# DixianZhu/deBWT

Hardware: AMD Instinct MI355X
Metric: Gbp/sec BWT build (30 Gbp synthetic DNA); bit-exact vs CPU ref; 1/2/4/8-GPU (higher is better)
Workload: dtype u64

## Files before the change

### debwt_amd/csrc/debwt_hip.hip

```cpp
#include "../../include/debwt_hip.h"

#include <hip/hip_runtime.h>

#include <algorithm>
#include <new>
#include <chrono>
#include <cmath>
#include <cstdio>
#include <cstring>
#include <atomic>
#include <string>
#include <thread>
#include <tuple>
#include <vector>

#include "radix_sort.h"
#include "special_host.h"
#include "fasta_host.h"
#include "gz_parallel.h"
#include "stage_kernels.h"
#include "special_kernels.h"
#include "verify_kernels.h"
#include "fm_kernels.h"
#include "fm_search_kernels.h"
// ... 1027 lines not shown
    }
    if ((rc = sync_check(c))) return rc;
    c->rB = c->h_scalars[4];
    c->rnlarge = c->h_scalars[5];
    c->rn1024 = c->h_scalars[11];
    c->rn512 = c->h_scalars[12];
    return DEBWT_OK;
}

static int append_range(debwt_ctx *c, debwt_ctx::KeyRange &r) {
    const u64 Q = c->rQ, nf = c->Rmo + Q;
    r.Q = Q; r.qbase = c->Q; r.B = c->rB; r.Bbase = c->B; r.l0 = c->nlarge; r.nl = c->rnlarge;
    ENSURE_KEEP(c, c->facts_acc, (c->nfacts_acc + nf) * 8 + 64, c->nfacts_acc * 8);
    ENSURE_KEEP(c, c->blk_j0, (c->Q + Q) * 8 + 64, c->Q * 8);
    ENSURE_KEEP(c, c->blk_freq, (c->Q + Q) * 4 + 64, c->Q * 4);
    ENSURE_KEEP(c, c->blk_start, (c->Q + Q) * 8 + 64, c->Q * 8);
    ENSURE_KEEP(c, c->large_q, (c->nlarge + c->rnlarge) * 4 + 64, c->nlarge * 4);
    if (nf) HIPCHK(c, hipMemcpyAsync(c->facts_acc.as<u64>() + c->nfacts_acc, c->facts.p, nf * 8, hipMemcpyDeviceToDevice, c->stream));
    if (Q)
        k_append_blocks<<<grid_for(Q, 256), 256, 0, c->stream>>>(c->mi_j0.as<u32>(), c->mi_freq.as<u32>(), c->bstart.as<u32>(), Q,
                                                                 r.Mbase, r.Bbase, c->blk_j0.as<u64>() + r.qbase,
                                                                 c->blk_freq.as<u32>() + r.qbase, c->blk_start.as<u64>() + r.qbase);
    if (c->rnlarge) {
        HIPCHK(c, hipMemcpyAsync(c->large_q.as<u32>() + c->nlarge, c->large_tmp.p, c->rnlarge * 4, hipMemcpyDeviceToDevice, c->stream));
        if (r.qbase)
            k_offset_u32<<<grid_for(c->rnlarge, 256), 256, 0, c->stream>>>(c->large_q.as<u32>() + c->nlarge, c->rnlarge, (u32)r.qbase);
    }
    c->nfacts_acc += nf; c->Q += Q; c->B += c->rB; c->nlarge += c->rnlarge; c->n1024 += c->rn1024; c->n512 += c->rn512;
    if (c->Q >= 0xFFFFFFF0ull) { c->err = "more than 2^32 multi-in blocks"; return DEBWT_ERANGE; }
    c->facts_ready = true;
    return sync_check(c);
}

static int classify_global(debwt_ctx *c, const u64 *d_facts, u64 nfacts, u64 qbase, u64 btotal) {
    const u64 nrec = c->nrec, Q = c->Q;
    int rc;
    const u64 nf = nfacts + nrec;
    c->nfacts = nf;
    c->qbase = qbase;
    c->Btotal = btotal;
    ENSURE(c, c->facts_all, nf * 8 + 64);
    ENSURE(c, c->facts_tmp, nf * 8 + 64);
    ENSURE(c, c->rs_skew, (nf / 2048 + 2) * 4);
    ENSURE(c, c->red, nf * 8 + 64);
    ENSURE(c, c->red_q, nf * 4 + 64);
    u64 *all = c->facts_all.as<u64>();
    if (nfacts) HIPCHK(c, hipMemcpyAsync(all, d_facts, nfacts * 8, hipMemcpyDeviceToDevice, c->stream));
    if (c->special_dev) HIPCHK(c, hipMemcpyAsync(all + nfacts, c->tail_d.p, nrec * 8, hipMemcpyDeviceToDevice, c->stream));
    else HIPCHK(c, hipMemcpyAsync(all + nfacts, c->special.tail_facts.data(), nrec * 8, hipMemcpyHostToDevice, c->stream));
    u64 *sorted_facts = nullptr;
    if ((rc = sort_keys(c, all, c->facts_tmp.as<u64>(), nf, 2 * c->cfg.k, &sorted_facts, false))) return rc;
    RedUniqueF fr{sorted_facts, nf, c->red.as<u64>()};
    if ((rc = cp_count(c, fr, nf, cp_area(c, 3), 3))) return rc;
    if ((rc = cp_emit(c, fr, nf, cp_area(c, 3)))) return rc;
    if ((rc = sync_check(c))) return rc;
    c->R = c->h_scalars[3];
    const u64 R = c->R;
    RedBlockF fq{c->red.as<u64>(), c->red_q.as<u32>()};
    if ((rc = cp_count(c, fq, R, cp_area(c, 6), 6))) return rc;
    if ((rc = cp_emit(c, fq, R, cp_area(c, 6)))) return rc;
    ENSURE(c, c->blue, c->B * 8 + 64);
    if ((rc = sync_check(c))) return rc;
    if (c->shard_world == 1 && c->h_scalars[6] != Q) {
        c->err = "multi-in count mismatch between fact list and red table";
        return DEBWT_EINTERNAL;
    }
    c->st.red_capacity = R; c->st.blue_capacity = c->B; c->st.blue_bound_num = Q; c->st.case3num = 2 * Q;
    c->st.blue_large_blocks = c->nlarge;
    c->Qtotal = c->h_scalars[6];
    c->stage = ST_CLASSIFIED;
    return DEBWT_OK;
}

extern "C" int debwt_classify(debwt_ctx *c) {
    if (!c) return DEBWT_EINVAL;
    if (c->stage < ST_SORTED) return DEBWT_ESTATE;
    if (c->shard_world > 1) { c->err = "sharded context: use debwt_shard_classify_local/_global"; return DEBWT_ESTATE; }
    HIPCHK(c, hipSetDevice(c->cfg.device));
    int rc;
    if (!c->local_done) {
        c->Q = c->B = c->nlarge = 0; c->nfacts_acc = 0; c->n1024 = 0; c->n512 = 0;
        if ((rc = classify_local(c))) return rc;
        if ((rc = append_range(c, c->ranges[0]))) return rc;
    }
    return classify_global(c, c->facts_acc.as<u64>(), c->nfacts_acc, 0, c->B);
}


static int sp_prepare(debwt_ctx *c) {
    HIPCHK(c, hipEventRecord(c->ev[4], c->stream));
    struct ReclaimScope { debwt_ctx *c; ~ReclaimScope() { c->reclaim_ok = false; } } rscope{c};
    c->reclaim_ok = true;
    const u64 ngroups = (c->n + 31) >> 5;
    ENSURE(c, c->momask, ngroups * 4 + 64);
    ENSURE(c, c->mimask, ngroups * 4 + 64);
    int hbits = 10;
    u64 slots_per_node = 4;
    if (const char *e = getenv("DEBWT_NODE_SLOTS")) slots_per_node = std::max<u64>(2, strtoull(e, nullptr, 10));
    while ((1ull << hbits) < slots_per_node * c->R) hbits++;
    if (hbits > 32 && (1ull << 32) >= 2 * c->R) hbits = 32;
    c->mzfilter = c->K >= 16 && !(c->cfg.reserved & 2048) && (hbits >= 20 || (c->cfg.reserved & 4096));
    c->mzw = c->K >= 24 ? MZ_W : MZ_W_SHORT;
    c->mztable = c->mzfilter && c->K >= 24 && (c->cfg.reserved & 16384);
    int pb;
    if (c->mzfilter) {
        pb = 10;
        while ((2ull << pb) < c->R) pb++;
        if (c->cfg.reserved & 15) pb += (c->cfg.reserved & 15) - 8;
        if (pb < 10) pb = 10;
        if (pb > 30) pb = 30;
    } else {
        pb = (c->cfg.reserved & 15) ? hbits + (c->cfg.reserved & 15) - 8
                                     : (hbits <= 24 ? std::max(hbits, std::min(hbits + 3, 24)) : hbits + 3);
        if (pb < 10) pb = 10;
        if (pb > 31) pb = 31;
    }
    if (pb > 31 || hbits > 32) { c->err = "more than 2^31 branching nodes: the node table has 2^32 slots"; return DEBWT_ERANGE; }
    c->hbits = hbits; c->pbits = pb;
    c->abs32 = c->B < 0xFFFFFFF0ull && !(c->cfg.reserved & 16);
    size_t rb_bytes = (c->mzfilter ? ((size_t)8 << pb) : ((size_t)1 << pb) / 8) + 64, ht_slots = (size_t)1 << hbits;
    ENSURE(c, c->rbits, rb_bytes);
    ENSURE(c, c->htab, ht_slots * sizeof(HSlot));
    HIPCHK(c, hipMemsetAsync(c->rbits.p, 0, rb_bytes, c->stream));
    HIPCHK(c, hipMemsetAsync(c->htab.p, 0, ht_slots * sizeof(HSlot), c->stream));
    if (c->R) {
        k_build_hash<<<grid_for(c->R, 256), 256, 0, c->stream>>>(c->red.as<u64>(), c->R, c->red_q.as<u32>(),
                                                                c->blk_start.as<u64>(), c->abs32 ? 1 : 0, (u32)c->qbase,
                                                                (u32)c->Q, hbits, c->htab.as<HSlot>(), c->mzfilter ? 0 : pb,
                                                                c->rbits.as<u32>(), c->mztable ? c->K : 0);
        if (c->mzfilter)
            k_build_mzfilter<<<grid_for(c->R, 256), 256, 0, c->stream>>>(c->red.as<u64>(), c->R, c->K, pb, c->rbits.as<u64>(), c->mzw);
    }
    return DEBWT_OK;
}

#define SP_SLICE_GROUPS (1ull << 26)
static SpBlockIds sp_block_ids(debwt_ctx *c) {
    if (!c->route_direct) return SpBlockIds{nullptr, nullptr, nullptr, 0};
    return SpBlockIds{c->qlist.as<u32>(), c->qwave.as<unsigned long long>(), c->qwave.as<u64>() + 1, c->gq0};
}
static int sp_block_ids_begin(debwt_ctx *c, u64 gq0, u64 groups) {
    c->route_direct = true; c->gq0 = gq0;
    ENSURE(c, c->qlist, (std::min<u64>(groups * 32, c->Btotal) + 64) * 4);
    ENSURE(c, c->qwave, ((groups + 63) / 64 + 2) * 8);
    HIPCHK(c, hipMemsetAsync(c->qwave.p, 0, 8, c->stream));
    return DEBWT_OK;
}

static int sp_flags(debwt_ctx *c, u64 g0, u64 g1) {
    int rc;
    if (g1 - g0 > (1ull << 27) - 2) { c->err = "text slice of the SP stage exceeds 2^32 positions"; return DEBWT_ERANGE; }
    c->g0 = g0; c->g1 = g1;
    const u64 ng = g1 - g0;
    if (ng && c->mzfilter && c->mztable)
        k_sp_flags<2><<<grid_for(ng, DEBWT_BLOCK), DEBWT_BLOCK, 0, c->stream>>>(
            c->text.as<u64>(), c->sepbits.as<u64>(), c->n, c->K, c->htab.as<HSlot>(), c->hbits, c->rbits.as<u32>(), c->pbits,
            c->branch.as<u64>(), c->nbranch, c->momask.as<u32>(), c->mimask.as<u32>(), g0, g1,
            sp_block_ids(c), c->branch_bitmap ? c->brbits.as<u64>() : nullptr);
    else if (ng && c->mzfilter)
        k_sp_flags<1><<<grid_for(ng, DEBWT_BLOCK), DEBWT_BLOCK, 0, c->stream>>>(
            c->text.as<u64>(), c->sepbits.as<u64>(), c->n, c->K, c->htab.as<HSlot>(), c->hbits, c->rbits.as<u32>(), c->pbits,
            c->branch.as<u64>(), c->nbranch, c->momask.as<u32>(), c->mimask.as<u32>(), g0, g1,
            sp_block_ids(c), c->branch_bitmap ? c->brbits.as<u64>() : nullptr, c->mzw);
    else if (ng)
        k_sp_flags<0><<<grid_for(ng, DEBWT_BLOCK), DEBWT_BLOCK, 0, c->stream>>>(
            c->text.as<u64>(), c->sepbits.as<u64>(), c->n, c->K, c->htab.as<HSlot>(), c->hbits, c->rbits.as<u32>(), c->pbits,
            c->branch.as<u64>(), c->nbranch, c->momask.as<u32>(), c->mimask.as<u32>(), g0, g1,
            sp_block_ids(c), c->branch_bitmap ? c->brbits.as<u64>() : nullptr);
    SpCountF fc{c->momask.as<u32>() + g0, c->mimask.as<u32>() + g0};
    if ((rc = cp_count2(c, fc, ng, cp_area(c, 0), 8, cp_area(c, 1), 10))) return rc;
    if ((rc = sync_check(c))) return rc;
    c->S_local = c->h_scalars[8];
    c->B_slice = c->h_scalars[10];
    return DEBWT_OK;
}

static int sp_emit(debwt_ctx *c, u64 sp_off, u64 *routed = nullptr, int qshift = 0) {
    const u64 ng = c->g1 - c->g0;
    c->sp_off = sp_off;
    ENSURE_KEEP(c, c->spsym, sp_off + c->S_local + 64, c->shard_world > 1 ? 0 : sp_off);
    if (!routed) ENSURE(c, c->mi_list, c->B_slice * 16 + 64);
    if (ng) {
        SpEmitArgs ea{c->text.as<u64>(), c->sepbits.as<u64>(), c->n, c->K, c->momask.as<u32>(), c->mimask.as<u32>(),
                      c->spsym.as<u8>(), routed ? nullptr : c->mi_list.as<ulonglong2>(), c->g0, sp_off,
                      routed, qshift, sp_block_ids(c)};
        u32 nchunks; u64 chunk;
        plan_chunks(ng, &nchunks, &chunk);
        k_sp_emit<<<nchunks, DEBWT_BLOCK, 0, c->stream>>>(ea, ng, chunk, cp_area(c, 0), cp_area(c, 1));
    }
    return DEBWT_OK;
}

static int sp_finish(debwt_ctx *c, u64 S) {
    c->S = S;
    u64 ntriples = (S >> 6) + 3;
    ENSURE(c, c->spn, ntriples * 24);
    k_pack_sp<<<grid_for(ntriples, 256), 256, 0, c->stream>>>(c->spsym.as<u8>(), S, ntriples, c->spn.as<u64>());
    c->st.sp_len = S;
    c->stage = ST_SP;
    return DEBWT_OK;
}

extern "C" int debwt_sp_generate(debwt_ctx *c) {
    if (!c) return DEBWT_EINVAL;
    if (c->stage < ST_CLASSIFIED) return DEBWT_ESTATE;
    HIPCHK(c, hipSetDevice(c->cfg.device));
    int rc;
    if ((rc = sp_prepare(c))) return rc;
    const u64 ngroups = (c->n + 31) >> 5;
    const u64 slice_groups = (c->cfg.reserved & 4194304) ? 4096ull : SP_SLICE_GROUPS;
    u64 S = 0, Bseen = 0;
    int qbits = 1;
    while ((1ull << qbits) < c->Q) qbits++;
    const int qshift = 64 - qbits;
    const bool route_sort = c->shard_world == 1 && c->Q > 0 && c->n < (1ull << (qshift - 3)) &&
                            c->B < 0xFFFFFFF0ull - (1ull << 20) &&
                            !(c->cfg.reserved & 32) &&
                            !((c->cfg.reserved & 262144) && c->ranges.size() > 1);
    const size_t P = c->ranges.size();
    bool route_ranges = !route_sort && c->shard_world == 1 && P > 1 && P <= RS_RADIX && c->Q > 0 && c->n < (1ull << (qshift - 3)) &&
                        !(c->cfg.reserved & 32);
    for (size_t i = 0; route_ranges && i < P; i++) route_ranges = c->ranges[i].B < 0xFFFFFFF0ull - (1ull << 20);
    std::vector<u64> rfill(P, 0), roffs(P + 1, 0);
    if (route_ranges) {
        std::vector<u32> qb(P + 1);
        for (size_t i = 0; i < P; i++) qb[i] = (u32)c->ranges[i].qbase;
        qb[P] = (u32)c->Q;
        ENSURE(c, c->qbounds, (P + 1) * 4);
        HIPCHK(c, hipMemcpyAsync(c->qbounds.p, qb.data(), (P + 1) * 4, hipMemcpyHostToDevice, c->stream));
        HIPCHK(c, hipStreamSynchronize(c->stream));
    }
    c->route_direct = false;
    for (u64 g0 = 0; g0 < ngroups; g0 += slice_groups) {
        const u64 g1 = std::min(ngroups, g0 + slice_groups);
        if ((route_sort || route_ranges) && (rc = sp_block_ids_begin(c, g0, g1 - g0))) return rc;
        if ((rc = sp_flags(c, g0, g1))) return rc;
        if (route_sort) {
            if (Bseen + c->B_slice > c->B) { c->err = "multi-in positions exceed the block total"; return DEBWT_EINTERNAL; }
            if ((rc = sp_emit(c, S, c->blue.as<u64>() + Bseen, qshift))) return rc;
        } else if (route_ranges) {
            u64 *ta = c->keysA.as<u64>(), *tb = c->keysB.as<u64>();
            size_t tb_cap = c->keysB.cap / 8;
            if (c->keysA.cap < c->B_slice * 8 + 64) { ENSURE(c, c->blue_tmp, c->B_slice * 8 + 64); ta = c->blue_tmp.as<u64>(); }
            if (c->keysB.cap < c->B_slice * 8 + 64) { ENSURE(c, c->mi_list, c->B_slice * 8 + 64); tb = c->mi_list.as<u64>(); tb_cap = c->mi_list.cap / 8; }
            if ((rc = sp_emit(c, S, ta, qshift))) return rc;
            if (c->B_slice) {
                ENSURE(c, c->rs_over, radix_over_bytes(c->B_slice));
                RsDigit dg{};
                dg.mode = 2; dg.bounds = c->qbounds.as<u32>(); dg.nb = (u32)P; dg.tshift = qshift;
                hipError_t e = radix_partition_by_shard(c->stream, ta, nullptr, c->B_slice, tb, dg, (u32)P, radix_ws(c), roffs.data(),
                                                        false, tb_cap);
                if (e != hipSuccess) { c->err = std::string("blue entries by key range: ") + hipGetErrorString(e); return DEBWT_EDEVICE; }
                for (size_t i = 0; i < P; i++) {
                    const u64 cnt = roffs[i + 1] - roffs[i];
                    if (!cnt) continue;
                    if (rfill[i] + cnt > c->ranges[i].B) { c->err = "multi-in positions exceed a key range's block total"; return DEBWT_EINTERNAL; }
                    HIPCHK(c, hipMemcpyAsync(c->blue.as<u64>() + c->ranges[i].Bbase + rfill[i], tb + roffs[i], cnt * 8,
                                             hipMemcpyDeviceToDevice, c->stream));
                    rfill[i] += cnt;
                }
            }
        } else if ((rc = sp_emit(c, S))) return rc;
        if (c->B_slice && !route_sort && !route_ranges) {
            if (c->abs32)
                k_blue_fill<1><<<grid_for(c->B_slice, DEBWT_BLOCK), DEBWT_BLOCK, 0, c->stream>>>(
                    c->mi_list.as<ulonglong2>(), c->B_slice, c->htab.as<HSlot>(), c->hbits, c->blk_start.as<u64>(),
                    (u32)c->qbase, c->blue.as<u64>(), c->mztable ? c->K : 0);
            else
                k_blue_fill<0><<<grid_for(c->B_slice, DEBWT_BLOCK), DEBWT_BLOCK, 0, c->stream>>>(
                    c->mi_list.as<ulonglong2>(), c->B_slice, c->htab.as<HSlot>(), c->hbits, c->blk_start.as<u64>(),
                    (u32)c->qbase, c->blue.as<u64>(), c->mztable ? c->K : 0);
        }
        S += c->S_local; Bseen += c->B_slice;
    }
    if (Bseen != c->Btotal) { c->err = "multi-in positions differ from the block total"; return DEBWT_EINTERNAL; }
    if (route_ranges) {
        for (size_t i = 0; i < P; i++) {
            const debwt_ctx::KeyRange &r = c->ranges[i];
            if (rfill[i] != r.B) { c->err = "multi-in positions differ from a key range's block total"; return DEBWT_EINTERNAL; }
            if (!r.B) continue;
            u64 *reg = c->blue.as<u64>() + r.Bbase, *res = reg;
            const int span = r.Q > 1 ? bits_for(r.qbase ^ (r.qbase + r.Q - 1)) : 0;
            bool stripped = false;
            if (span) {
                ENSURE(c, c->rs_over, radix_over_bytes(r.B));
                ENSURE(c, c->rs_pair, radix_pair_bytes(r.B, qshift, std::min(64, qshift + span), true, nullptr));
                u64 *tmp = c->keysA.as<u64>();
                if (c->keysA.cap < r.B * 8 + 64) { ENSURE(c, c->blue_tmp, r.B * 8 + 64); tmp = c->blue_tmp.as<u64>(); }
                hipError_t e = hipSuccess;
                u64 *third = c->keysB.cap >= r.B * 8 + 64 && c->keysB.as<u64>() != tmp ? c->keysB.as<u64>() : nullptr;
                res = radix_sort_bits(c->stream, reg, tmp, r.B, qshift, std::min(64, qshift + span), radix_ws(c), &e, qshift, &stripped, third);
                if (e != hipSuccess) { c->err = std::string("blue entry sort: ") + hipGetErrorString(e); return DEBWT_EDEVICE; }
            }
            if (!stripped) k_blue_strip<<<grid_for(r.B, 256), 256, 0, c->stream>>>(res, reg, r.B, qshift);
        }
    }
    if (route_sort && c->B) {
        u64 *tmp;
        if (c->keysA.cap >= c->B * 8) tmp = c->keysA.as<u64>();
        else { ENSURE(c, c->blue_tmp, c->B * 8 + 64); tmp = c->blue_tmp.as<u64>(); }
        ENSURE(c, c->rs_over, radix_over_bytes(c->B));
        ENSURE(c, c->rs_pair, radix_pair_bytes(c->B, qshift, 64, true, nullptr));
        hipError_t e = hipSuccess;
        bool stripped = false;
        u64 *third = c->keysB.cap >= c->B * 8 + 64 && c->keysB.as<u64>() != tmp ? c->keysB.as<u64>() : nullptr;
        u64 *r = radix_sort_bits(c->stream, c->blue.as<u64>(), tmp, c->B, qshift, 64, radix_ws(c), &e, qshift, &stripped, third);
        if (e != hipSuccess) { c->err = std::string("blue entry sort: ") + hipGetErrorString(e); return DEBWT_EDEVICE; }
        if (!stripped) k_blue_strip<<<grid_for(c->B, 256), 256, 0, c->stream>>>(r, c->blue.as<u64>(), c->B, qshift);
    }
    return sp_finish(c, S);
}


static int bitonic_large(debwt_ctx *c, u64 b0, u32 m, u64 j0) {
    u64 P = 2;
    while (P < m) P <<= 1;
    ENSURE(c, c->large_k0, P * 8);
    ENSURE(c, c->large_en, P * 8);
    k_large_load<<<grid_for(P, 256), 256, 0, c->stream>>>(c->blue.as<u64>(), b0, m, P, c->spn.as<u64>(),
                                                          c->large_k0.as<u64>(), c->large_en.as<u64>());
    for (u64 kk = 2; kk <= P; kk <<= 1)
// ... 5891 lines not shown
```

### debwt_amd/csrc/stage_kernels.h

```cpp
#pragma once
#include "common.h"


#ifndef CP_MAXCHUNKS
#define CP_MAXCHUNKS 2048
#endif

#define CP_VEC 4

template <class F>
__global__ __launch_bounds__(DEBWT_BLOCK) void cp_count_kernel(F f, u64 n, u64 chunk, u32 *__restrict__ counts) {
    __shared__ u32 red[DEBWT_WAVES];
    u64 beg = (u64)blockIdx.x * chunk;
    u64 end = beg + chunk < n ? beg + chunk : n;
    u32 local = 0;
    for (u64 i = beg + threadIdx.x; i < end; i += DEBWT_BLOCK * CP_VEC) {
#pragma unroll
        for (int v = 0; v < CP_VEC; v++)
            if (i + (u64)v * DEBWT_BLOCK < end) local += f.count(i + (u64)v * DEBWT_BLOCK);
    }
    u32 incl = wave_scan_incl(local);
    if (lane_id() == 63) red[threadIdx.x >> 6] = incl;
    __syncthreads();
    if (threadIdx.x == 0) {
// ... 438 lines not shown
    blk_start[q] = bbase + bstart[q];
}
__global__ void k_count_blocks(const u32 *__restrict__ mi_freq, u64 Q, u32 lo, u32 hi, u32 *__restrict__ counter) {
    u32 n = 0;
    for (u64 q = (u64)blockIdx.x * blockDim.x + threadIdx.x; q < Q; q += (u64)gridDim.x * blockDim.x) {
        const u32 f = mi_freq[q];
        n += (f > lo && f <= hi) ? 1u : 0u;
    }
#pragma unroll
    for (int d = 32; d >= 1; d >>= 1) n += __shfl_xor(n, d, 64);
    if (n && (threadIdx.x & 63u) == 0) atomicAdd(counter, n);
}
__global__ void k_offset_u32(u32 *__restrict__ v, u64 n, u32 add) {
    u64 i = (u64)blockIdx.x * blockDim.x + threadIdx.x;
    if (i < n) v[i] += add;
}

struct __attribute__((aligned(16))) HSlot {
    u64 key;
    u32 cur;
    u32 q;
};
#define HCURSOR_SKIP 0xFFFFFFFFu
__device__ __forceinline__ u32 hmask(int hbits) { return hbits >= 32 ? 0xFFFFFFFFu : (1u << hbits) - 1u; }
__device__ __forceinline__ u32 red_hash(u64 node, int bits) { return (u32)((node * 0x9E3779B97F4A7C15ull) >> (64 - bits)); }
__device__ __forceinline__ u32 red_hash2(u64 node, int bits) { return (u32)((node * 0xC2B2AE3D27D4EB4Full) >> (64 - bits)); }

#define MZ_W 16
__device__ __forceinline__ u32 mz_hash(u32 x) { x *= 0x9E3779B1u; x ^= x >> 15; return x * 0x85EBCA6Bu; }
__device__ __forceinline__ u32 mz_word(u32 m, int fbits) { return (m * 0xC2B2AE3Du) >> (32 - fbits); }
__device__ __forceinline__ u32 mz_bit(u64 node) { return (u32)((node * 0xC2B2AE3D27D4EB4Full) >> 58); }
__device__ __forceinline__ u32 mz_pair(u32 m, u32 o, int hbits) { return (((m * 0x27D4EB2Fu) >> (32 - (hbits - 5))) << 5) + 2u * o; }
#define MZ_W_SHORT 12
__device__ __forceinline__ u32 mz_of_node(u64 node, int K, u32 *off, int mzw = MZ_W) {
    const u64 win = node << (64 - 2 * K);
    const int nw = K - mzw + 1, hs = 32 - 2 * mzw;
    u32 m = 0xFFFFFFFFu, o = 0;
    for (int j = 0; j < nw; j++) {
        const u32 h = mz_hash((u32)(win >> (32 - 2 * j)) >> hs);
        if (h < m) { m = h; o = (u32)j; }
    }
    *off = o;
    return m;
}

__global__ void k_build_hash(const u64 *__restrict__ red, u64 R, const u32 *__restrict__ red_q,
                             const u64 *__restrict__ blk_start, int abs32, u32 qbase, u32 Qlocal, int hbits,
                             HSlot *__restrict__ htab, int pb, u32 *__restrict__ rbits, int mzK) {
    u64 r = (u64)blockIdx.x * blockDim.x + threadIdx.x;
    if (r >= R) return;
    const u64 v = red[r], node = v >> 2;
    const u32 mask = hmask(hbits);
    u32 h = 0;
    bool placed = false;
    if (mzK) {
        u32 o;
        const u32 m = mz_of_node(node, mzK, &o);
        h = mz_pair(m, o, hbits);
        placed = atomicCAS(&htab[h].key, 0ull, v) == 0ull;
        if (!placed) placed = atomicCAS(&htab[++h].key, 0ull, v) == 0ull;
    }
    if (!placed) {
        h = red_hash(node, hbits);
        for (;;) {
            u64 old = atomicCAS(&htab[h].key, 0ull, v);
            if (old == 0ull) break;
            h = (h + 1) & mask;
        }
    }
    if (v & 2ull) {
        u32 q = red_q[r] - qbase;
        htab[h].cur = q < Qlocal ? (abs32 ? (u32)blk_start[q] : 0u) : HCURSOR_SKIP;
        htab[h].q = red_q[r];
    }
    if (pb) {
        u32 hb = red_hash2(node, pb);
        atomicOr(&rbits[hb >> 5], 1u << (hb & 31));
    }
}

__global__ void k_build_mzfilter(const u64 *__restrict__ red, u64 R, int K, int fbits, u64 *__restrict__ fw, int mzw) {
    u64 r = (u64)blockIdx.x * blockDim.x + threadIdx.x;
    if (r >= R) return;
    const u64 node = red[r] >> 2;
    u32 o;
    atomicOr(&fw[mz_word(mz_of_node(node, K, &o, mzw), fbits)], 1ull << mz_bit(node));
}

__device__ __forceinline__ u32 red_lookup(const HSlot *__restrict__ htab, int hbits, u64 node, u32 *flags, int mzK = 0) {
    const u32 mask = hmask(hbits);
    if (mzK) {
        u32 o;
        const u32 m = mz_of_node(node, mzK, &o);
        const u32 a = mz_pair(m, o, hbits);
        for (u32 h = a; h < a + 2u; h++) {
            const u64 v = htab[h].key;
            if (v == 0ull) { *flags = 0; return 0xFFFFFFFFu; }
            if ((v >> 2) == node) { *flags = (u32)(v & 3); return h; }
        }
    }
    u32 h = red_hash(node, hbits);
    for (;;) {
        u64 v = htab[h].key;
        if (v == 0ull) { *flags = 0; return 0xFFFFFFFFu; }
        if ((v >> 2) == node) { *flags = (u32)(v & 3); return h; }
        h = (h + 1) & mask;
    }
}

__device__ __forceinline__ u32 red_lookup_q(const HSlot *__restrict__ htab, int hbits, u64 node, u32 *q) {
    const u32 mask = hmask(hbits);
    u32 h = red_hash(node, hbits);
    for (;;) {
        const ulonglong2 v = *reinterpret_cast<const ulonglong2 *>(&htab[h]);
        if (v.x == 0ull) return 0u;
        if ((v.x >> 2) == node) { *q = (u32)(v.y >> 32); return (u32)(v.x & 3); }
        h = (h + 1) & mask;
    }
}
__device__ __forceinline__ u32 red_lookup_q_mz(const HSlot *__restrict__ htab, int hbits, u64 node, u32 a, u32 *q) {
    const ulonglong2 v0 = *reinterpret_cast<const ulonglong2 *>(&htab[a]);
    const ulonglong2 v1 = *reinterpret_cast<const ulonglong2 *>(&htab[a + 1u]);
    if ((v0.x >> 2) == node && v0.x) { *q = (u32)(v0.y >> 32); return (u32)(v0.x & 3); }
    if ((v1.x >> 2) == node && v1.x) { *q = (u32)(v1.y >> 32); return (u32)(v1.x & 3); }
    if (v0.x == 0ull || v1.x == 0ull) return 0u;
    return red_lookup_q(htab, hbits, node, q);
}

__global__ void k_special_rows(const u64 *__restrict__ dk, const u32 *__restrict__ dstart, u64 D, u64 M,
                               const u64 *__restrict__ spkey, u64 NS, u64 row_base, u64 *__restrict__ sprow) {
    u64 s = (u64)blockIdx.x * blockDim.x + threadIdx.x;
    if (s >= NS) return;
    const u64 e = upper_bound_dev<u64>(dk, 0, D, (spkey[s] << 2) | 3ull);
    sprow[s] = row_base + s + (e < D ? (u64)dstart[e] : M);
}


struct SpBlockIds {
    u32 *list;
    unsigned long long *count;
    u64 *wave_base;
    u64 g0;
};

#ifndef SP_FLAGS_WAVES
#define SP_FLAGS_WAVES 4
#endif
#ifndef SP_EMIT_STAGE
#define SP_EMIT_STAGE 1
#endif
#ifndef SP_PROBE_BATCH
#define SP_PROBE_BATCH 2
#endif
template <int MZ>
__global__ __launch_bounds__(DEBWT_BLOCK) __attribute__((amdgpu_waves_per_eu(SP_FLAGS_WAVES))) void k_sp_flags(const u64 *__restrict__ text, const u64 *__restrict__ sepbits,
                                                           u64 n, int K, const HSlot *__restrict__ htab, int hbits,
                                                           const u32 *__restrict__ rbits, int pb,
                                                           const u64 *__restrict__ branch, u64 nbranch,
                                                           u32 *__restrict__ momask, u32 *__restrict__ mimask,
                                                           u64 g0, u64 g1, SpBlockIds ids, const u64 *__restrict__ brbits, int mzw = MZ_W) {
    __shared__ u32 lq[DEBWT_BLOCK * 32];
    u64 g = g0 + (u64)blockIdx.x * blockDim.x + threadIdx.x;
    const bool active = g < g1;
    if (!ids.list && !active) return;
    u32 mo = 0, mi = 0;
    if (active) {
    const u64 w0 = text[g], w1 = text[g + 1];
    const u64 sb = sep_window(sepbits, g << 5);
    const u64 i0 = g << 5;
    u32 lim = (n - i0) < 32 ? (u32)(n - i0) : 32u;
    const u32 inrange = lim == 32 ? 0xFFFFFFFFu : ((1u << lim) - 1u);
    u32 cand = 0, spec = 0;
    if (MZ) {
        const u64 *fw = reinterpret_cast<const u64 *>(rbits);
        const int nw = K - mzw + 1, hs = 32 - 2 * mzw;
        u32 H[47];
#pragma unroll
        for (int j = 0; j < 47; j++) {
            u32 x;
            if (j <= 16) x = (u32)(w0 >> (32 - 2 * j));
            else if (j < 32) x = (u32)(w0 << (2 * j - 32)) | (u32)(w1 >> (96 - 2 * j));
            else x = (u32)(w1 >> (96 - 2 * j));
            H[j] = mz_hash(x >> hs);
        }
        u32 mprev = 0;
        u64 fwv = 0;
#pragma unroll
        for (u32 t = 0; t < 32; t++) {
            u32 m = H[t], o = 0;
#pragma unroll
            for (int d = 1; d < 16; d++)
                if (d < nw) {
                    const bool lt = H[t + d] < m;
                    m = lt ? H[t + d] : m;
                    if (MZ == 2) o = lt ? (u32)d : o;
                }
            if (t == 0 || m != mprev) fwv = fw[mz_word(m, pb)];
            mprev = m;
            const u64 win = t ? ((w0 << (2 * t)) | (w1 >> (64 - 2 * t))) : w0;
            const u32 bit = (u32)((fwv >> mz_bit(win >> (64 - 2 * K))) & 1ull);
            if (MZ == 2 && bit) lq[threadIdx.x * 32 + t] = mz_pair(m, o, hbits);
            cand |= bit << t;
        }
    } else {
#pragma unroll
    for (u32 t = 0; t < 32; t++) {
        u64 win = t ? ((w0 << (2 * t)) | (w1 >> (64 - 2 * t))) : w0;
        u32 hb = red_hash2(win >> (64 - 2 * K), pb);
        u32 bit = (rbits[hb >> 5] >> (hb & 31)) & 1u;
        cand |= bit << t;
    }
    }
    if (wave_any(sb != 0ull)) spec = sep_blocked(sb, K);
    cand &= inrange & ~spec;
    spec &= inrange;
    if (MZ == 2) {
        constexpr int SP_BATCH = 4;
        while (cand) {
            u32 tt[SP_BATCH], ad[SP_BATCH];
            u64 nd[SP_BATCH];
            ulonglong2 v0[SP_BATCH], v1[SP_BATCH];
            bool have[SP_BATCH];
#pragma unroll
            for (int b = 0; b < SP_BATCH; b++) {
                have[b] = cand != 0u;
                const u32 t = have[b] ? (u32)__ffs(cand) - 1u : 0u;
                cand &= cand - 1u;
                tt[b] = t;
                nd[b] = (t ? ((w0 << (2 * t)) | (w1 >> (64 - 2 * t))) : w0) >> (64 - 2 * K);
                ad[b] = lq[threadIdx.x * 32 + t];
            }
#pragma unroll
            for (int b = 0; b < SP_BATCH; b++) {
                v0[b] = v1[b] = make_ulonglong2(0ull, 0ull);
                if (have[b]) {
                    v0[b] = *reinterpret_cast<const ulonglong2 *>(&htab[ad[b]]);
                    v1[b] = *reinterpret_cast<const ulonglong2 *>(&htab[ad[b] + 1u]);
                }
            }
#pragma unroll
            for (int b = 0; b < SP_BATCH; b++) {
                if (!have[b]) continue;
                u32 fl = 0, q = 0;
                if (v0[b].x && (v0[b].x >> 2) == nd[b]) { fl = (u32)(v0[b].x & 3ull); q = (u32)(v0[b].y >> 32); }
                else if (v1[b].x && (v1[b].x >> 2) == nd[b]) { fl = (u32)(v1[b].x & 3ull); q = (u32)(v1[b].y >> 32); }
                else if (v0[b].x && v1[b].x) fl = red_lookup_q(htab, hbits, nd[b], &q);
                mo |= (fl & 1u) << tt[b];
                mi |= ((fl >> 1) & 1u) << tt[b];
                if (ids.list && (fl & 2u)) lq[threadIdx.x * 32 + tt[b]] = q;
            }
        }
    }
#if SP_PROBE_BATCH > 1
    while (cand) {
        u32 tt[SP_PROBE_BATCH], hh[SP_PROBE_BATCH];
        u64 nd[SP_PROBE_BATCH];
        ulonglong2 v[SP_PROBE_BATCH];
        bool have[SP_PROBE_BATCH];
#pragma unroll
        for (int b = 0; b < SP_PROBE_BATCH; b++) {
            have[b] = cand != 0u;
            const u32 t = have[b] ? (u32)__ffs(cand) - 1u : 0u;
            cand &= cand - 1u;
            tt[b] = t;
            nd[b] = (t ? ((w0 << (2 * t)) | (w1 >> (64 - 2 * t))) : w0) >> (64 - 2 * K);
            hh[b] = red_hash(nd[b], hbits);
        }
#pragma unroll
        for (int b = 0; b < SP_PROBE_BATCH; b++) {
            v[b] = make_ulonglong2(0ull, 0ull);
            if (have[b]) v[b] = *reinterpret_cast<const ulonglong2 *>(&htab[hh[b]]);
        }
#pragma unroll
        for (int b = 0; b < SP_PROBE_BATCH; b++) {
            if (!have[b] || v[b].x == 0ull) continue;
            u32 fl, q = 0;
            if ((v[b].x >> 2) == nd[b]) { fl = (u32)(v[b].x & 3ull); q = (u32)(v[b].y >> 32); }
            else {
                const u32 mask = hmask(hbits);
                u32 h = (hh[b] + 1u) & mask;
                fl = 0;
                for (;;) {
                    const ulonglong2 x = *reinterpret_cast<const ulonglong2 *>(&htab[h]);
                    if (x.x == 0ull) break;
                    if ((x.x >> 2) == nd[b]) { fl = (u32)(x.x & 3ull); q = (u32)(x.y >> 32); break; }
                    h = (h + 1u) & mask;
                }
            }
            mo |= (fl & 1u) << tt[b];
            mi |= ((fl >> 1) & 1u) << tt[b];
            if (ids.list && (fl & 2u)) lq[threadIdx.x * 32 + tt[b]] = q;
        }
    }
#else
    while (cand) {
        u32 t = (u32)__ffs(cand) - 1u;
        cand &= cand - 1u;
        u64 win = t ? ((w0 << (2 * t)) | (w1 >> (64 - 2 * t))) : w0;
        u32 q = 0;
        const u32 fl = red_lookup_q(htab, hbits, win >> (64 - 2 * K), &q);
        mo |= (fl & 1u) << t;
        mi |= ((fl >> 1) & 1u) << t;
        if (ids.list && (fl & 2u)) lq[threadIdx.x * 32 + t] = q;
    }
#endif
    if (brbits) {
        if (spec) mo |= (u32)sep_window(brbits, i0) & spec;
    } else if (nbranch) {
        while (spec) {
            u32 t = (u32)__ffs(spec) - 1u;
            spec &= spec - 1u;
            u64 i = i0 + t;
            u64 lo = lower_bound_dev<u64>(branch, 0, nbranch, i);
            if (lo < nbranch && branch[lo] == i) mo |= 1u << t;
        }
    }
    momask[g] = mo;
    mimask[g] = mi;
    }
    if (!ids.list) return;
    const u32 cnt = (u32)__popc(mi);
    u32 incl = cnt;
#pragma unroll
    for (int d = 1; d < 64; d <<= 1) {
        const u32 v = __shfl_up(incl, d, 64);
        if ((int)lane_id() >= d) incl += v;
    }
    const u32 total = __shfl(incl, 63, 64);
    u64 base = 0;
    if (lane_id() == 0 && total) base = atomicAdd(ids.count, (unsigned long long)total);
    base = ((u64)__shfl((u32)(base >> 32), 0, 64) << 32) | __shfl((u32)base, 0, 64);
    if (lane_id() == 0 && active) ids.wave_base[(g - ids.g0) >> 6] = base;
    u64 o = base + incl - cnt;
    while (mi) {
        const u32 t = (u32)__ffs(mi) - 1u;
        mi &= mi - 1u;
        ids.list[o++] = lq[threadIdx.x * 32 + t];
    }
}

struct SpCountF {
    const u32 *momask; const u32 *mimask;
    __device__ void count2(u64 g, u32 *a, u32 *b) const { *a = (u32)__popc(momask[g]); *b = (u32)__popc(mimask[g]); }
};
struct SpEmitArgs {
    const u64 *text; const u64 *sepbits; u64 n; int K;
    const u32 *momask; const u32 *mimask;
    u8 *spsym; ulonglong2 *mi_list;
    u64 g0;
    u64 sp_base;
    u64 *routed; int qshift; SpBlockIds ids;
};
__global__ __launch_bounds__(DEBWT_BLOCK) void k_sp_emit(SpEmitArgs a, u64 ngroups, u64 chunk,
                                                          const u32 *__restrict__ off_mo,
                                                          const u32 *__restrict__ off_mi) {
// ... 1277 lines not shown
```

Measured before the change: 24.32.

## Batch minimizer filter-word loads in SP flags kernel via LDS staging

Restructures the minimizer-filter path of k_sp_flags. It first records the distinct minimizer values per thread into a rotated LDS scratch area, then issues the filter-word global loads in batches of FB so several are in flight at once, then resolves each position's bit from the staged words. Previously each load was a dependent gather issued serially inside the 32-position loop. Minimizer offsets are packed into registers and the hashes for the lq pairs are recomputed afterwards. This adds LDS traffic, extra passes when more than 16 minimizers change, and more code complexity. A reserved config bit selects an FB=1 variant, and the host launch is unified through a kernel function pointer.

```diff
diff --git a/debwt_amd/csrc/debwt_hip.hip b/debwt_amd/csrc/debwt_hip.hip
--- a/debwt_amd/csrc/debwt_hip.hip
+++ b/debwt_amd/csrc/debwt_hip.hip
@@ -1203,21 +1203,16 @@
     if (g1 - g0 > (1ull << 27) - 2) { c->err = "text slice of the SP stage exceeds 2^32 positions"; return DEBWT_ERANGE; }
     c->g0 = g0; c->g1 = g1;
     const u64 ng = g1 - g0;
-    if (ng && c->mzfilter && c->mztable)
-        k_sp_flags<2><<<grid_for(ng, DEBWT_BLOCK), DEBWT_BLOCK, 0, c->stream>>>(
-            c->text.as<u64>(), c->sepbits.as<u64>(), c->n, c->K, c->htab.as<HSlot>(), c->hbits, c->rbits.as<u32>(), c->pbits,
-            c->branch.as<u64>(), c->nbranch, c->momask.as<u32>(), c->mimask.as<u32>(), g0, g1,
-            sp_block_ids(c), c->branch_bitmap ? c->brbits.as<u64>() : nullptr);
-    else if (ng && c->mzfilter)
-        k_sp_flags<1><<<grid_for(ng, DEBWT_BLOCK), DEBWT_BLOCK, 0, c->stream>>>(
+    auto *kern = &k_sp_flags<0>;
+    if (c->mzfilter) {
+        const bool one = (c->cfg.reserved & 33554432) != 0;
+        kern = c->mztable ? (one ? &k_sp_flags<2, 1> : &k_sp_flags<2>) : (one ? &k_sp_flags<1, 1> : &k_sp_flags<1>);
+    }
+    if (ng)
+        kern<<<grid_for(ng, DEBWT_BLOCK), DEBWT_BLOCK, 0, c->stream>>>(
             c->text.as<u64>(), c->sepbits.as<u64>(), c->n, c->K, c->htab.as<HSlot>(), c->hbits, c->rbits.as<u32>(), c->pbits,
             c->branch.as<u64>(), c->nbranch, c->momask.as<u32>(), c->mimask.as<u32>(), g0, g1,
             sp_block_ids(c), c->branch_bitmap ? c->brbits.as<u64>() : nullptr, c->mzw);
-    else if (ng)
-        k_sp_flags<0><<<grid_for(ng, DEBWT_BLOCK), DEBWT_BLOCK, 0, c->stream>>>(
-            c->text.as<u64>(), c->sepbits.as<u64>(), c->n, c->K, c->htab.as<HSlot>(), c->hbits, c->rbits.as<u32>(), c->pbits,
-            c->branch.as<u64>(), c->nbranch, c->momask.as<u32>(), c->mimask.as<u32>(), g0, g1,
-            sp_block_ids(c), c->branch_bitmap ? c->brbits.as<u64>() : nullptr);
     SpCountF fc{c->momask.as<u32>() + g0, c->mimask.as<u32>() + g0};
     if ((rc = cp_count2(c, fc, ng, cp_area(c, 0), 8, cp_area(c, 1), 10))) return rc;
     if ((rc = sync_check(c))) return rc;
diff --git a/debwt_amd/csrc/stage_kernels.h b/debwt_amd/csrc/stage_kernels.h
--- a/debwt_amd/csrc/stage_kernels.h
+++ b/debwt_amd/csrc/stage_kernels.h
@@ -614,14 +614,17 @@
 #ifndef SP_PROBE_BATCH
 #define SP_PROBE_BATCH 2
 #endif
-template <int MZ>
+#ifndef SP_FILTER_BATCH
+#define SP_FILTER_BATCH 4
+#endif
+template <int MZ, int FB = SP_FILTER_BATCH>
 __global__ __launch_bounds__(DEBWT_BLOCK) __attribute__((amdgpu_waves_per_eu(SP_FLAGS_WAVES))) void k_sp_flags(const u64 *__restrict__ text, const u64 *__restrict__ sepbits,
                                                            u64 n, int K, const HSlot *__restrict__ htab, int hbits,
                                                            const u32 *__restrict__ rbits, int pb,
                                                            const u64 *__restrict__ branch, u64 nbranch,
                                                            u32 *__restrict__ momask, u32 *__restrict__ mimask,
                                                            u64 g0, u64 g1, SpBlockIds ids, const u64 *__restrict__ brbits, int mzw = MZ_W) {
-    __shared__ u32 lq[DEBWT_BLOCK * 32];
+    __shared__ __attribute__((aligned(8))) u32 lq[DEBWT_BLOCK * 32];
     u64 g = g0 + (u64)blockIdx.x * blockDim.x + threadIdx.x;
     const bool active = g < g1;
     if (!ids.list && !active) return;
@@ -636,33 +639,74 @@
     if (MZ) {
         const u64 *fw = reinterpret_cast<const u64 *>(rbits);
         const int nw = K - mzw + 1, hs = 32 - 2 * mzw;
-        u32 H[47];
-#pragma unroll
-        for (int j = 0; j < 47; j++) {
-            u32 x;
-            if (j <= 16) x = (u32)(w0 >> (32 - 2 * j));
-            else if (j < 32) x = (u32)(w0 << (2 * j - 32)) | (u32)(w1 >> (96 - 2 * j));
-            else x = (u32)(w1 >> (96 - 2 * j));
-            H[j] = mz_hash(x >> hs);
-        }
-        u32 mprev = 0;
-        u64 fwv = 0;
-#pragma unroll
-        for (u32 t = 0; t < 32; t++) {
-            u32 m = H[t], o = 0;
-#pragma unroll
-            for (int d = 1; d < 16; d++)
-                if (d < nw) {
-                    const bool lt = H[t + d] < m;
-                    m = lt ? H[t + d] : m;
-                    if (MZ == 2) o = lt ? (u32)d : o;
-                }
-            if (t == 0 || m != mprev) fwv = fw[mz_word(m, pb)];
-            mprev = m;
-            const u64 win = t ? ((w0 << (2 * t)) | (w1 >> (64 - 2 * t))) : w0;
-            const u32 bit = (u32)((fwv >> mz_bit(win >> (64 - 2 * K))) & 1ull);
-            if (MZ == 2 && bit) lq[threadIdx.x * 32 + t] = mz_pair(m, o, hbits);
-            cand |= bit << t;
+        static_assert(16 % FB == 0, "a pass of 16 change points is a whole number of trips");
+        u32 *const lm = &lq[threadIdx.x * 32];
+        const u32 rot = 2u * threadIdx.x;
+        u32 O[4] = {0u, 0u, 0u, 0u};
+        for (u32 base = 0;; base += 16) {
+            u64 x0 = w0, x1 = w1;
+            asm volatile("" : "+v"(x0), "+v"(x1));
+            u32 H[47];
+#pragma unroll
+            for (int j = 0; j < 47; j++) {
+                u32 x;
+                if (j <= 16) x = (u32)(x0 >> (32 - 2 * j));
+                else if (j < 32) x = (u32)(x0 << (2 * j - 32)) | (u32)(x1 >> (96 - 2 * j));
+                else x = (u32)(x1 >> (96 - 2 * j));
+                H[j] = mz_hash(x >> hs);
+            }
+            u32 mprev = 0, chg = 0, c = 0u - 1u - base;
+#pragma unroll
+            for (u32 t = 0; t < 32; t++) {
+                u32 m = H[t], o = 0;
+#pragma unroll
+                for (int d = 1; d < 16; d++)
+                    if (d < nw) {
+                        const bool lt = H[t + d] < m;
+                        m = lt ? H[t + d] : m;
+                        if (MZ == 2) o = lt ? (u32)d : o;
+                    }
+                const u32 ch = (t == 0 || m != mprev) ? 1u : 0u;
+                mprev = m;
+                chg |= ch << t;
+                c += ch;
+                lm[((c < 16u ? 16u + c : 0u) + rot) & 31u] = m;
+                if (MZ == 2) O[t >> 3] |= o << (4 * (t & 7));
+            }
+            if (MZ == 2) asm volatile("" : "+v"(O[0]), "+v"(O[1]), "+v"(O[2]), "+v"(O[3]));
+            const u32 nchg = (u32)__popc(chg);
+            const u32 nv = nchg > base ? (nchg - base < 16u ? nchg - base : 16u) : 0u;
+            for (u32 j = 0; wave_any(j < nv); j += FB) {
+                u32 a[FB];
+                u64 w[FB];
+#pragma unroll
+                for (int b = 0; b < FB; b++) {
+                    const u32 mc = lm[(16u + j + b + rot) & 31u];
+                    a[b] = mz_word(j + b < nv ? mc : mprev, pb);
+                }
+#pragma unroll
+                for (int b = 0; b < FB; b++) w[b] = fw[a[b]];
+#pragma unroll
+                for (int b = 0; b < FB; b++) *reinterpret_cast<u64 *>(&lm[(2u * (j + b) + rot) & 31u]) = w[b];
+            }
+#pragma unroll
+            for (u32 t = 0; t < 32; t++) {
+                const u32 ct = (u32)__popc(chg & ((2u << t) - 1u)) - 1u - base;
+                const u64 fwv = *reinterpret_cast<const u64 *>(&lm[(2u * (ct & 15u) + rot) & 31u]);
+                const u64 win = t ? ((x0 << (2 * t)) | (x1 >> (64 - 2 * t))) : x0;
+                const u32 bit = (u32)((fwv >> mz_bit(win >> (64 - 2 * K))) & 1ull);
+                cand |= (ct < 16u ? bit : 0u) << t;
+            }
+            if (!wave_any(nchg > base + 16u)) break;
+        }
+        if (MZ == 2) {
+#pragma unroll
+            for (u32 t = 0; t < 32; t++)
+                if ((cand >> t) & 1u) {
+                    const u32 o = (O[t >> 3] >> (4 * (t & 7))) & 15u, j = t + o;
+                    const u64 at = j < 32 ? (j ? ((w0 << (2 * j)) | (w1 >> (64 - 2 * j))) : w0) : (w1 << (2 * j - 64));
+                    lq[threadIdx.x * 32 + t] = mz_pair(mz_hash((u32)(at >> 32) >> hs), o, hbits);
+                }
         }
     } else {
 #pragma unroll
```

Result: no change. 24.43 (median of 6 runs) (+0.5%).
